# dcherednik/atracdenc

Hardware: AMD Instinct MI355X
Metric: ATRAC3 1024-sample stereo frames/sec (higher is better)
Workload: dtype f32; 1 GPU; ATRAC3 LP2 132 kbps stereo, 64 streams x 64 frames = 4096 frames per GPU per step (BASELINE configs[1]), 'noise' PCM resident in HBM, frames written to HBM (PCIe excluded); streams_per_gpu=64, frame_bytes=384, input=noise, tonal_components=True, parallelism=streams/1, launch=1 process x 1 GPU(s), one host thread and one at3hip context per device, collectives=none (no RCCL); start/stop barrier only

## Files before the change

atracdenc_amd/csrc/at3_k_gain.hpp:

```cpp
#pragma once
#include "at3_common.hpp"

namespace at3 {

struct GainParams {
    const float* sub;
    GainRec* rec;
    cpx* bins;
    BandState* state;
    Curve* curves;
    int n_blocks;
    int f0;
    int js;
    int n_streams;
    int literal;
};

constexpr int kLowCutBin = 38;

__device__ inline void median3_32(const float* in, float* out)
{
    for (int i = 0; i < 32; ++i) {
        const int lo = i > 0 ? i - 1 : 0;
        const int hi = i < 31 ? i + 1 : 31;
        if (hi - lo == 1) {
            out[i] = fmaxf(in[lo], in[hi]);
        } else {
            const float a = in[lo], b = in[lo + 1], c = in[hi];
            out[i] = fmaxf(fminf(a, b), fminf(fmaxf(a, b), c));
        }
    }
}

__device__ inline float curve_target(const float* in, const float* filtered)
{
    float maxRaw = 0.0f;
    for (int i = 0; i < 32; ++i) maxRaw = fmaxf(maxRaw, in[i]);
    float bestLevel = 0.0f;
    int bestEnd = -1;
    for (int j = 0; j + 3 <= 32; ++j) {
        const float minVal = fminf(fminf(filtered[j], filtered[j + 1]), filtered[j + 2]);
        if (minVal > bestLevel) {
            bestLevel = minVal;
            bestEnd = j + 2;
        }
    }
    float plateau = 0.0f;
    bool release = false;
    if (!(bestLevel < 1e-6f)) {
        plateau = bestLevel;
        while (bestEnd + 1 < 32 && filtered[bestEnd + 1] >= bestLevel) ++bestEnd;
        if (bestEnd < 31) {
            if (in[31] < bestLevel * 0.1f) {
                release = true;
            } else {
                bool anyHigh = false;
                for (int i = bestEnd + 1; i < 32; ++i)
                    if (in[i] >= bestLevel * 0.7f) {
                        anyHigh = true;
                        break;
                    }
                release = !anyHigh && (in[31] < bestLevel * 0.5f);
            }
        }
    }
    const bool usePlateau = plateau > 1e-6f && !release && plateau >= maxRaw * 0.4f;
    return usePlateau ? plateau : in[31];
}

__device__ __forceinline__ int irfft_pad(int i) { return i + (i >> 5); }

template <bool Z1>
__device__ __forceinline__ void bfly4_inv_sparse(f2& x0, f2& x1, f2& x2, f2& x3, f2 w1, f2 w3)
{
    const f2 s2 = pk_cmul(x3, w3);
    const f2 f0 = x0;
    if (Z1) {
        x2 = f0 - s2;
        x0 = f0 + s2;
        x1 = pk_sub_ib(f0, s2);
        x3 = pk_add_ib(f0, s2);
    } else {
        const f2 s0 = pk_cmul(x1, w1);
        const f2 s3 = s0 + s2, s4 = s0 - s2;
        x2 = f0 - s3;
        x0 = f0 + s3;
        x1 = pk_add_ib(f0, s4);
        x3 = pk_sub_ib(f0, s4);
    }
}

template <int KAPPA>
__device__ __forceinline__ void irfft_pass_2_8(cpx* F, const cpx* tw, int lane)
{
    cpx* B = F + 33 * lane + KAPPA;
    f2 x[16];
    const int r0 = (lane >> 4) + 4 * ((lane >> 2) & 3) + 16 * (lane & 3);
#pragma unroll
    for (int i = 0; i < 16; ++i) {
        const int r = r0 + 64 * (i >> 2);
        const bool nz = (i & 3) == 0 ? r >= 38 : (i & 3) == 1 ? r == 0 : (i & 3) == 3 ? r <= 218 : false;
        x[i] = f2{0.0f, 0.0f};
        if ((i & 3) != 2 && nz) x[i] = ld2(B + 2 * i);
    }
    const f2 a1 = ld2(tw + 256 * KAPPA), a3 = ld2(tw + 768 * KAPPA);
    bfly4_inv_sparse<false>(x[0], x[1], x[2], x[3], a1, a3);
#pragma unroll
    for (int g = 1; g < 4; ++g) bfly4_inv_sparse<true>(x[4 * g], x[4 * g + 1], x[4 * g + 2], x[4 * g + 3], a1, a3);
#pragma unroll
    for (int j = 0; j < 4; ++j) {
        const int k = KAPPA + 2 * j;
        bfly4<true>(x[j], x[j + 4], x[j + 8], x[j + 12], ld2(tw + 64 * k), ld2(tw + 128 * k), ld2(tw + 192 * k));
    }
#pragma unroll
    for (int i = 0; i < 16; ++i) st2(B + 2 * i, x[i]);
}

struct Tw32_128 {
    f2 a[3];
    f2 w[4][3];
};
__device__ __forceinline__ Tw32_128 irfft_tw_32_128(const cpx (*g)[128], int v)
{
    Tw32_128 t;
    t.a[0] = ld2(&g[0][v]);
    t.a[1] = ld2(&g[1][v]);
    t.a[2] = ld2(&g[2][v]);
#pragma unroll
    for (int j = 0; j < 4; ++j) {
        t.w[j][0] = ld2(&g[3 + 3 * j][v]);
        t.w[j][1] = ld2(&g[4 + 3 * j][v]);
        t.w[j][2] = ld2(&g[5 + 3 * j][v]);
    }
    return t;
}
__device__ __forceinline__ void irfft_pass_32_128(cpx* F, const Tw32_128& t, int v)
{
    const int k = v & 31, G2 = v >> 5;
    cpx* B = F + 528 * G2 + k;
    f2 x[16];
#pragma unroll
    for (int i = 0; i < 16; ++i) x[i] = ld2(B + 33 * i);
#pragma unroll
    for (int g = 0; g < 4; ++g) bfly4<true>(x[4 * g], x[4 * g + 1], x[4 * g + 2], x[4 * g + 3], t.a[0], t.a[1], t.a[2]);
#pragma unroll
    for (int j = 0; j < 4; ++j) bfly4<true>(x[j], x[j + 4], x[j + 8], x[j + 12], t.w[j][0], t.w[j][1], t.w[j][2]);
#pragma unroll
    for (int i = 0; i < 16; ++i) st2(B + 33 * i, x[i]);
}

template <int NT>
struct Tw512 {
    f2 w[512 / NT][3];
};
template <int NT>
__device__ __forceinline__ Tw512<NT> irfft_tw_512(const cpx (*g)[128], int tid)
{
    static_assert(NT == 128, "Tables::gain_tw is laid out for 128 work-items");
    Tw512<NT> t;
#pragma unroll
    for (int u = 0; u < 512 / NT; ++u) {
        t.w[u][0] = ld2(&g[15 + 3 * u][tid]);
        t.w[u][1] = ld2(&g[16 + 3 * u][tid]);
        t.w[u][2] = ld2(&g[17 + 3 * u][tid]);
    }
    return t;
}
template <int NT>
__device__ __forceinline__ void irfft_pass_512(cpx* F, const Tw512<NT>& t, int tid)
{
#pragma unroll
    for (int u0 = 0; u0 < 512 / NT; u0 += 4) {
        f2 x[4][4];
        cpx* B[4];
#pragma unroll
        for (int u = 0; u < 4; ++u) {
            B[u] = F + irfft_pad(tid + NT * (u0 + u));
#pragma unroll
            for (int q = 0; q < 4; ++q) x[u][q] = ld2(B[u] + 528 * q);
        }
#pragma unroll
        for (int u = 0; u < 4; ++u) bfly4<true>(x[u][0], x[u][1], x[u][2], x[u][3], t.w[u0 + u][0], t.w[u0 + u][1], t.w[u0 + u][2]);
#pragma unroll
        for (int u = 0; u < 4; ++u) {
            st2(B[u] + 528, x[u][1]);
            st2(B[u] + 1056, x[u][2]);
        }
    }
}

template <int CTRL>
__device__ __forceinline__ double dpp_f64_zero_fill(double v)
{
    const uint64_t b = (uint64_t)__double_as_longlong(v);
    const uint32_t lo = (uint32_t)AT3_DPP((uint32_t)b, CTRL, true), hi = (uint32_t)AT3_DPP((uint32_t)(b >> 32), CTRL, true);
    return __longlong_as_double((long long)(((uint64_t)hi << 32) | lo));
}
__device__ __forceinline__ double row_scan_add_f64(double v)
{
    v += dpp_f64_zero_fill<0x111>(v);
    v += dpp_f64_zero_fill<0x112>(v);
    v += dpp_f64_zero_fill<0x114>(v);
    v += dpp_f64_zero_fill<0x118>(v);
    return v;
}
constexpr int kGainBins = 220;

constexpr int kSpecRowStride = 18;
constexpr int kSpecItemBytes = 2432;
struct SpecItemLds {
    union {
        cpx x[16 * kSpecRowStride];
        double e[304];
    };
};
static_assert(sizeof(SpecItemLds) == kSpecItemBytes, "SpecItemLds layout");

__global__ __launch_bounds__(64) void k_gain_spec(GainParams p, const Tables* T, int n_items)
{
    __shared__ __attribute__((aligned(16))) SpecItemLds s_item[4];
    const int lane = threadIdx.x, row = lane >> 4, L = lane & 15;
    SpecItemLds& S = s_item[row];
    const int nfr = p.n_blocks - p.f0;
    const int quads = (nfr + 3) >> 2;
    int wg = blockIdx.x;
    const int band = wg % 3; wg /= 3;
    const int ch = wg % 2; wg /= 2;
    const int fr = 4 * (wg % quads) + row;
    const int s = wg / quads;
    const bool valid = fr < nfr;
    const int f = p.f0 + (valid ? fr : nfr - 1);
    const int item = (((s * nfr) + (f - p.f0)) * 2 + ch) * 3 + band;
    (void)n_items;
    const int cb = f - 1;
    const size_t sublen = (size_t)(p.n_blocks + 2) * 256;
    const float* sb0 = p.sub + ((size_t)s * 8 + 0 * 4 + band) * sublen + (size_t)(cb + 2) * 256 - 128;
    const float* sb1 = p.sub + ((size_t)s * 8 + 1 * 4 + band) * sublen + (size_t)(cb + 2) * 256 - 128;
    GainRec* rec = p.rec + (((size_t)s * p.n_blocks + f) * 2 + ch) * 3 + band;
    cpx* bins = p.bins + (size_t)item * kGainBins;

    f2 a[16];
    {
        f2 raw[16], rb[16], win[16];
#pragma unroll
        for (int t = 0; t < 16; ++t) {
            const int i = L + 16 * t;
            raw[t] = *reinterpret_cast<const f2*>((p.js || ch == 0 ? sb0 : sb1) + 2 * i);
            if (p.js) rb[t] = *reinterpret_cast<const f2*>(sb1 + 2 * i);
        }
#pragma unroll
        for (int t = 0; t < 16; ++t) win[t] = ld2(&T->spec16_win[t][L]);
        __builtin_amdgcn_sched_barrier(0);
#pragma unroll
        for (int t = 0; t < 16; ++t) {
            f2 v = raw[t];
            if (p.js) v = (ch == 0) ? (v + rb[t]) * mk2(0.5f, 0.5f) : (v - rb[t]) * mk2(0.5f, 0.5f);
            a[4 * (t & 3) + (t >> 2)] = v * win[t];
        }
    }
    f2 tw_l[15];
#pragma unroll
    for (int q = 0; q < 15; ++q) tw_l[q] = ld2(&T->spec16_tw[q][L]);
    __builtin_amdgcn_sched_barrier(0);
    {
        const f2 w0 = ld2(&T->tw256[0]);
#pragma unroll
        for (int q3 = 0; q3 < 4; ++q3) bfly4<false>(a[4 * q3], a[4 * q3 + 1], a[4 * q3 + 2], a[4 * q3 + 3], w0, w0, w0);
#pragma unroll
        for (int k = 0; k < 4; ++k)
            bfly4<false>(a[k], a[k + 4], a[k + 8], a[k + 12], ld2(&T->tw256[16 * k]), ld2(&T->tw256[32 * k]), ld2(&T->tw256[48 * k]));
    }
    f2 b[16];
    {
#pragma unroll
        for (int r = 0; r < 16; ++r) st2(&S.x[r * kSpecRowStride + L], a[r]);
        wave_sync();
        const float4* src = reinterpret_cast<const float4*>(&S.x[L * kSpecRowStride]);
#pragma unroll
        for (int m = 0; m < 8; ++m) {
            const float4 v = src[m];
            b[2 * m] = mk2(v.x, v.y);
            b[2 * m + 1] = mk2(v.z, v.w);
        }
        wave_sync();
    }
    {
        const f2 u1 = tw_l[0], u2 = tw_l[1], u3 = tw_l[2];
#pragma unroll
        for (int q1 = 0; q1 < 4; ++q1) bfly4<false>(b[q1], b[q1 + 4], b[q1 + 8], b[q1 + 12], u1, u2, u3);
#pragma unroll
        for (int j = 0; j < 4; ++j) bfly4<false>(b[4 * j], b[4 * j + 1], b[4 * j + 2], b[4 * j + 3], tw_l[3 + 3 * j], tw_l[4 + 3 * j], tw_l[5 + 3 * j]);
    }
    f2 fa[8], fb[8];
    f2 f128 = mk2(0.0f, 0.0f);
    {
        const int partner = 4 * ((lane & 48) | ((16 - L) & 15));
#pragma unroll
        for (int jj = 0; jj < 8; ++jj) {
            const int je = 15 - jj;
            const f2 pe = b[(je >> 2) + 4 * (je & 3)];
            f2 other;
            other.x = __uint_as_float((uint32_t)__builtin_amdgcn_ds_bpermute(partner, (int)__float_as_uint(pe.x)));
            other.y = __uint_as_float((uint32_t)__builtin_amdgcn_ds_bpermute(partner, (int)__float_as_uint(pe.y)));
            if (jj > 0) {
                const int j0 = 16 - jj;
                const f2 own = b[(j0 >> 2) + 4 * (j0 & 3)];
                if (L == 0) other = own;
            }
            const f2 fpk = b[(jj >> 2) + 4 * (jj & 3)];
            const cpx stw = T->spec16_stw[jj][L];
            const float fnr = other.x, fni = -other.y;
            const float f1r = fpk.x + fnr, f1i = fpk.y + fni;
            const float f2r = fpk.x - fnr, f2i = fpk.y - fni;
            const float twr = f2r * stw.r - f2i * stw.i, twi = f2r * stw.i + f2i * stw.r;
            fa[jj] = mk2((f1r + twr) * 0.5f, (f1i + twi) * 0.5f);
            fb[jj] = mk2((f1r - twr) * 0.5f, (twi - f1i) * 0.5f);
        }
        if (L == 0) {
            const f2 f0 = b[0];
            fa[0] = mk2(f0.x + f0.y, 0.0f);
            fb[0] = mk2(f0.x - f0.y, 0.0f);
        }
        {
            const f2 fpk = b[2];
            const cpx stw = T->spec16_stw[8][L];
            const float fnr = fpk.x, fni = -fpk.y;
            const float f1r = fpk.x + fnr, f1i = fpk.y + fni;
            const float f2r = fpk.x - fnr, f2i = fpk.y - fni;
            const float twr = f2r * stw.r - f2i * stw.i, twi = f2r * stw.i + f2i * stw.r;
            f128 = mk2((f1r - twr) * 0.5f, (twi - f1i) * 0.5f);
        }
    }
    if (valid) {
#pragma unroll
        for (int jj = 0; jj < 8; ++jj) {
            const int k = L + 16 * jj;
            if (k >= kLowCutBin) st2(&bins[k - kLowCutBin], fa[jj]);
            st2(&bins[256 - k - kLowCutBin], fb[jj]);
        }
        if (L == 0) st2(&bins[128 - kLowCutBin], f128);
    }
    bool fast_done = false;
    {
        const double h1 = (double)T->hpf_w[1], h2 = (double)T->hpf_w[2];
        double et = 0.0, ef = 0.0;
#pragma unroll
        for (int jj = 0; jj < 8; ++jj) {
            const int k = L + 16 * jj;
            const double ea = (double)fa[jj].x * fa[jj].x + (double)fa[jj].y * fa[jj].y;
            const double eb = (double)fb[jj].x * fb[jj].x + (double)fb[jj].y * fb[jj].y;
            et += ea;
            et += eb;
            const double wa = (k < kLowCutBin) ? 0.0 : (k == kLowCutBin) ? ea * h1 * h1 : (k == kLowCutBin + 1) ? ea * h2 * h2 : ea;
            ef += wa;
            ef += eb;
        }
        if (L == 0) {
            const double e128 = (double)f128.x * f128.x + (double)f128.y * f128.y;
            et += e128;
            ef += e128;
        }
        et = row_scan_add_f64(et);
        ef = row_scan_add_f64(ef);
        bool need = false;
        float hfr = 0.0f;
        if (L == 15) {
            if (et > 0.0 && ef > 0.0) {
                const double r = ef / et;
                hfr = (float)r;
                if (!(hfr >= 1e-30f)) {
                    need = true;
                } else {
                    const uint32_t hb = __float_as_uint(hfr);
                    const double below = ((double)__uint_as_float(hb - 1u) + (double)hfr) * 0.5, above = ((double)hfr + (double)__uint_as_float(hb + 1u)) * 0.5;
                    const double margin = r * 4e-13;
                    need = !(r - below > margin && above - r > margin);
                }
            }
        }
        if (p.literal || __ballot(need && valid) != 0ull) {
            fast_done = false;
        } else {
            if (valid && L == 15) rec->hfr = hfr;
            fast_done = true;
        }
    }
    if (fast_done) return;
    {
#pragma unroll
        for (int jj = 0; jj < 8; ++jj) {
            const int k = L + 16 * jj;
            S.e[k] = (double)fa[jj].x * fa[jj].x + (double)fa[jj].y * fa[jj].y;
            S.e[256 - k] = (double)fb[jj].x * fb[jj].x + (double)fb[jj].y * fb[jj].y;
        }
        if (L == 0) S.e[128] = (double)f128.x * f128.x + (double)f128.y * f128.y;
        for (int k = 257 + L; k < 304; k += 16) S.e[k] = 0.0;
    }
    wave_sync();
    double acc = 0.0;
    if (lane < 8) {
        const int it = lane >> 1, kind = lane & 1;
        const double* E = s_item[it].e;
        const double h1 = (double)T->hpf_w[1], h2 = (double)T->hpf_w[2];
        if (kind == 1) {
            acc += E[kLowCutBin] * h1 * h1;
            acc += E[kLowCutBin + 1] * h2 * h2;
        }
        const double* src = E + (kind ? kLowCutBin + 2 : 0);
        for (int k0 = 0; k0 < 256; k0 += 16) {
            double v[16];
#pragma unroll
            for (int i = 0; i < 16; ++i) v[i] = src[k0 + i];
#pragma unroll
            for (int i = 0; i < 16; ++i) acc += v[i];
        }
        acc += src[256];
    }
    const uint64_t ab = (uint64_t)__double_as_longlong(acc);
    const int alo = (int)(uint32_t)ab, ahi = (int)(uint32_t)(ab >> 32);
    const uint64_t fb64 = (uint64_t)(uint32_t)__builtin_amdgcn_ds_bpermute(4 * (2 * row + 1), alo) |
                          ((uint64_t)(uint32_t)__builtin_amdgcn_ds_bpermute(4 * (2 * row + 1), ahi) << 32);
    const uint64_t tb64 = (uint64_t)(uint32_t)__builtin_amdgcn_ds_bpermute(4 * (2 * row), alo) |
                          ((uint64_t)(uint32_t)__builtin_amdgcn_ds_bpermute(4 * (2 * row), ahi) << 32);
    if (valid && L == 0) {
        const double totalE = __longlong_as_double((long long)tb64), filtE = __longlong_as_double((long long)fb64);
        rec->hfr = (totalE > 0.0) ? (float)(filtE / totalE) : 0.0f;
    }
}

struct GainLds {
    cpx f[2048 + 64];
};

__global__ __launch_bounds__(128) void k_gain_analysis(GainParams p, const Tables* __restrict__ T)
{
    __shared__ __attribute__((aligned(16))) GainLds s_item[1];
    const int tid = threadIdx.x, wave = __builtin_amdgcn_readfirstlane((int)(threadIdx.x >> 6)), lane = threadIdx.x & 63;
    GainLds& L = s_item[0];
    const int nfr = p.n_blocks - p.f0;
    const bool valid = true;
    int wg = blockIdx.x;
    const size_t item = blockIdx.x;
    const int band = wg % 3; wg /= 3;
    const int ch = wg % 2; wg /= 2;
    const int f = p.f0 + wg % nfr;
    const int s = wg / nfr;
    GainRec* rec = p.rec + (((size_t)s * p.n_blocks + f) * 2 + ch) * 3 + band;
    const float hfr = rec->hfr;
    const cpx* bins = p.bins + item * kGainBins;
    const int k0 = kLowCutBin + tid, k1 = kLowCutBin + 128 + tid;
    const cpx bin0 = bins[tid];
    const cpx bin1 = bins[k1 <= 256 ? 128 + tid : tid];
    const cpx stw_in0 = T->stw2048[k0 - 1];
    const cpx stw_in1 = T->stw2048[k1 - 1 < 1024 ? k1 - 1 : 1023];
    const float hpf1 = T->hpf_w[1], hpf2 = T->hpf_w[2];
    __builtin_amdgcn_sched_barrier(0);
    if (hfr < 0.05f) return;
    __builtin_amdgcn_sched_barrier(0);
    const Tw32_128 tw_b = irfft_tw_32_128(T->gain_tw, tid);
    const Tw512<128> tw_c = irfft_tw_512<128>(T->gain_tw, tid);
    __builtin_amdgcn_sched_barrier(0);
#pragma unroll
    for (int q = 0; q < 2; ++q) {
        const int k = q ? k1 : k0;
        const cpx fr = q ? bin1 : bin0;
        cpx fk;
        const float scale = 8.0f;
        if (k == 256) {
            fk.r = fr.r * scale * 0.5f;
            fk.i = 0.0f;
        } else if (k >= kLowCutBin + 2) {
            fk.r = fr.r * scale;
            fk.i = fr.i * scale;
        } else {
            const float w = (k == kLowCutBin) ? hpf1 : hpf2;
            fk.r = fr.r * scale * w;
            fk.i = fr.i * scale * w;
        }
        const cpx fok = cmul(fk, q ? stw_in1 : stw_in0);
        cpx a, b, nb;
        a.r = fk.r + fok.r; a.i = fk.i + fok.i;
        b.r = fk.r - fok.r; b.i = -(fk.i - fok.i);
        nb.r = 0.0f - b.r; nb.i = 0.0f - b.i;
        if (k <= 256) {
            const int pa = fft_leaf_pos<2048>(k);
            L.f[irfft_pad(pa)] = a;
            L.f[irfft_pad(pa) + 1] = a;
            const int pb = fft_leaf_pos<2048>(2048 - k);
            L.f[irfft_pad(pb) - 1] = b;
            L.f[irfft_pad(pb)] = nb;
        }
    }
    __syncthreads();

    if (wave == 0) irfft_pass_2_8<0>(L.f, T->tw2048, lane);
    else irfft_pass_2_8<1>(L.f, T->tw2048, lane);
    __syncthreads();

    irfft_pass_32_128(L.f, tw_b, tid);
    __syncthreads();

    irfft_pass_512<128>(L.f, tw_c, tid);
    __syncthreads();


    const float norm = 1.0f / 4096.0f;
    float* s_micro = reinterpret_cast<float*>(L.f);
#pragma unroll
    for (int q = 0; q < 2; ++q) {
        const int n = tid + 128 * q;
        const int c = (n & 3) | ((n & 0xc) << 1) | ((n & 0x10) >> 2) | (n & 0xe0);
        cpx* src = L.f + 528 + 4 * c + (c >> 3);
        float acc = 0.0f;
#pragma unroll
        for (int i = 0; i < 4; ++i) {
            const f2 v = ld2(src + i) * norm;
            const f2 sq = v * v;
            st2(src + i, sq);
            acc += sq.x;
            acc += sq.y;
        }
        acc /= 8;
        s_micro[c] = sqrtf(acc);
    }
    __syncthreads();
    if (tid < 32) {
        const cpx* src = L.f + 528 + 33 * lane;
        f2 x[32];
#pragma unroll
        for (int i = 0; i < 32; ++i) x[i] = ld2(src + i);
        float acc = 0.0f;
#pragma unroll
        for (int i = 0; i < 32; ++i) {
            acc += x[i].x;
            acc += x[i].y;
        }
        acc /= 64;
        rec->gain[lane] = sqrtf(acc);
    } else if (wave == 1 && lane < 32) {
        const float4 ma = *reinterpret_cast<const float4*>(s_micro + 8 * lane), mb = *reinterpret_cast<const float4*>(s_micro + 8 * lane + 4);
        float m[8] = {ma.x, ma.y, ma.z, ma.w, mb.x, mb.y, mb.z, mb.w};
#pragma unroll
        for (int i = 1; i < 8; ++i) {
#pragma unroll
            for (int k = i; k > 0; --k) {
                const float lo = fminf(m[k - 1], m[k]), hi = fmaxf(m[k - 1], m[k]);
                m[k - 1] = lo;
                m[k] = hi;
            }
        }
        rec->lo[lane] = m[2];
        rec->hi[lane] = m[6];
    }
}

constexpr int kGa1RowStride = 18;
constexpr int kGa1RowSlots = 16 * kGa1RowStride + 16;
constexpr int kGa1SubStride = 33;
struct Gain1Lds {
    union {
        cpx x[4 * kGa1RowSlots];
        struct {
            cpx out[32 * kGa1SubStride];
            float micro[256];
        };
    };
};
static_assert(sizeof(Gain1Lds) <= 10240, "sixteen items per CU");

struct PermPair {
    int a, b;
};
__device__ __forceinline__ PermPair perm32_swap(int a, int b)
{
    const auto r = __builtin_amdgcn_permlane32_swap(a, b, false, false);
    return PermPair{(int)r[0], (int)r[1]};
}
__device__ __forceinline__ PermPair perm16_swap(int a, int b)
{
    const auto r = __builtin_amdgcn_permlane16_swap(a, b, false, false);
    return PermPair{(int)r[0], (int)r[1]};
}
template <bool WIDE>
__device__ __forceinline__ void swap_f2(f2& a, f2& b)
{
    const PermPair x = WIDE ? perm32_swap((int)__float_as_uint(a.x), (int)__float_as_uint(b.x)) : perm16_swap((int)__float_as_uint(a.x), (int)__float_as_uint(b.x));
    const PermPair y = WIDE ? perm32_swap((int)__float_as_uint(a.y), (int)__float_as_uint(b.y)) : perm16_swap((int)__float_as_uint(a.y), (int)__float_as_uint(b.y));
    a = mk2(__uint_as_float((uint32_t)x.a), __uint_as_float((uint32_t)y.a));
    b = mk2(__uint_as_float((uint32_t)x.b), __uint_as_float((uint32_t)y.b));
}

__global__ __launch_bounds__(64) AT3_WAVES_PER_EU(4) void k_gain_analysis1(GainParams p, const Tables* T)
{
    __shared__ __attribute__((aligned(16))) Gain1Lds L;
    const int lane = threadIdx.x, R = lane >> 4, j = lane & 15;
    const int nfr = p.n_blocks - p.f0;
    int wg = blockIdx.x;
    const size_t item = blockIdx.x;
    const int band = wg % 3; wg /= 3;
    const int ch = wg % 2; wg /= 2;
    const int f = p.f0 + wg % nfr;
    const int s = wg / nfr;
    GainRec* rec = p.rec + (((size_t)s * p.n_blocks + f) * 2 + ch) * 3 + band;
    const float hfr = rec->hfr;
    if (hfr < 0.05f) return;
    const cpx* bins = p.bins + item * kGainBins;
    const cpx* tw = T->tw2048;

#define AT3_STAGE() __builtin_amdgcn_sched_barrier(0)
    const int r0 = (lane >> 4) + 4 * ((lane >> 2) & 3) + 16 * (lane & 3);
    cpx ba[4], bb[4], sa[4], sb[4], b256 = {0.0f, 0.0f}, s256 = {0.0f, 0.0f};
#pragma unroll
    for (int q = 0; q < 4; ++q) {
        const int ka = r0 + 64 * q, kb = 256 - r0 - 64 * q;
        const int kac = ka >= kLowCutBin ? ka : kLowCutBin, kbc = kb >= kLowCutBin ? kb : kLowCutBin;
        ba[q] = bins[kac - kLowCutBin];
        sa[q] = T->stw2048[kac - 1];
        bb[q] = bins[kbc - kLowCutBin];
        sb[q] = T->stw2048[kbc - 1];
    }
    if (lane == 0) {
        b256 = bins[256 - kLowCutBin];
        s256 = T->stw2048[255];
    }
    const float hpf1 = T->hpf_w[1], hpf2 = T->hpf_w[2];
    f2 a1[2], a3[2], w8[2][4][3];
#pragma unroll
    for (int kappa = 0; kappa < 2; ++kappa) {
        a1[kappa] = ld2(tw + 256 * kappa);
        a3[kappa] = ld2(tw + 768 * kappa);
#pragma unroll
        for (int jj = 0; jj < 4; ++jj) {
            const int k = kappa + 2 * jj;
            w8[kappa][jj][0] = ld2(tw + 64 * k);
            w8[kappa][jj][1] = ld2(tw + 128 * k);
            w8[kappa][jj][2] = ld2(tw + 192 * k);
        }
    }
    f2 twb[15];
#pragma unroll
    for (int sl = 0; sl < 15; ++sl) twb[sl] = ld2(&T->ga1_twb[0][sl][j]);
    AT3_STAGE();
    f2 la[4], lb[4], la256 = mk2(0.0f, 0.0f);
    {
        auto leaf = [&](cpx fr, cpx stw, int k, bool want_b) -> f2 {
            cpx fk;
            const float scale = 8.0f;
            if (k == 256) {
                fk.r = fr.r * scale * 0.5f;
                fk.i = 0.0f;
            } else if (k >= kLowCutBin + 2) {
                fk.r = fr.r * scale;
                fk.i = fr.i * scale;
            } else {
                const float w = (k == kLowCutBin) ? hpf1 : hpf2;
                fk.r = fr.r * scale * w;
                fk.i = fr.i * scale * w;
            }
            const cpx fok = cmul(fk, stw);
            return want_b ? mk2(fk.r - fok.r, -(fk.i - fok.i)) : mk2(fk.r + fok.r, fk.i + fok.i);
        };
#pragma unroll
        for (int q = 0; q < 4; ++q) {
            const int ka = r0 + 64 * q, kb = 256 - r0 - 64 * q;
            la[q] = (ka >= kLowCutBin) ? leaf(ba[q], sa[q], ka, false) : mk2(0.0f, 0.0f);
            lb[q] = (kb >= kLowCutBin) ? leaf(bb[q], sb[q], kb, true) : mk2(0.0f, 0.0f);
        }
        if (lane == 0) la256 = leaf(b256, s256, 256, false);
    }
    f2 y[2][16];
    f2 twc[2][4][3];
#pragma unroll
    for (int kappa = 0; kappa < 2; ++kappa) {
        f2 x[16];
#pragma unroll
        for (int i = 0; i < 16; ++i) x[i] = mk2(0.0f, 0.0f);
#pragma unroll
        for (int q = 0; q < 4; ++q) {
            x[4 * q] = la[q];
            x[4 * q + 3] = kappa ? mk2(0.0f - lb[q].x, 0.0f - lb[q].y) : lb[q];
        }
        x[1] = la256;
        bfly4_inv_sparse<false>(x[0], x[1], x[2], x[3], a1[kappa], a3[kappa]);
#pragma unroll
        for (int g = 1; g < 4; ++g) bfly4_inv_sparse<true>(x[4 * g], x[4 * g + 1], x[4 * g + 2], x[4 * g + 3], a1[kappa], a3[kappa]);
#pragma unroll
        for (int jj = 0; jj < 4; ++jj) bfly4<true>(x[jj], x[jj + 4], x[jj + 8], x[jj + 12], w8[kappa][jj][0], w8[kappa][jj][1], w8[kappa][jj][2]);
        cpx* row = L.x + R * kGa1RowSlots;
#pragma unroll
        for (int i = 0; i < 16; ++i) st2(row + i * kGa1RowStride + j, x[i]);
        wave_sync();
        f2 b[16];
        {
            const float4* src = reinterpret_cast<const float4*>(row + j * kGa1RowStride);
#pragma unroll
            for (int m = 0; m < 8; ++m) {
                const float4 v = src[m];
                b[2 * m] = mk2(v.x, v.y);
                b[2 * m + 1] = mk2(v.z, v.w);
            }
        }
        wave_sync();
#pragma unroll
        for (int g = 0; g < 4; ++g) bfly4<true>(b[4 * g], b[4 * g + 1], b[4 * g + 2], b[4 * g + 3], twb[0], twb[1], twb[2]);
#pragma unroll
        for (int jj = 0; jj < 4; ++jj) bfly4<true>(b[jj], b[jj + 4], b[jj + 8], b[jj + 12], twb[3 + 3 * jj], twb[4 + 3 * jj], twb[5 + 3 * jj]);
#pragma unroll
        for (int i = 0; i < 16; ++i) y[kappa][i] = b[i];
        AT3_STAGE();
        if (kappa == 0) {
#pragma unroll
            for (int sl = 0; sl < 15; ++sl) twb[sl] = ld2(&T->ga1_twb[1][sl][j]);
        } else {
#pragma unroll
            for (int u = 0; u < 2; ++u)
#pragma unroll
                for (int t = 0; t < 4; ++t)
#pragma unroll
                    for (int q = 0; q < 3; ++q) twc[u][t][q] = ld2(&T->ga1_twc[4 * u + t][q][lane]);
        }
        AT3_STAGE();
    }
#pragma unroll
    for (int u = 0; u < 2; ++u)
#pragma unroll
        for (int t = 0; t < 8; ++t) swap_f2<true>(y[u][t], y[u][8 + t]);
#pragma unroll
    for (int u = 0; u < 2; ++u)
#pragma unroll
        for (int t = 0; t < 4; ++t) {
            swap_f2<false>(y[u][t], y[u][4 + t]);
            swap_f2<false>(y[u][8 + t], y[u][12 + t]);
        }
#pragma unroll
    for (int u = 0; u < 2; ++u)
#pragma unroll
        for (int t = 0; t < 4; ++t) {
            const int i = 4 * R + t;
            bfly4<true>(y[u][t], y[u][4 + t], y[u][8 + t], y[u][12 + t], twc[u][t][0], twc[u][t][1], twc[u][t][2]);
            st2(L.out + kGa1SubStride * i + 2 * j + u, y[u][4 + t]);
            st2(L.out + kGa1SubStride * (16 + i) + 2 * j + u, y[u][8 + t]);
        }
    wave_sync();
    const float norm = 1.0f / 4096.0f;
#pragma unroll
    for (int q = 0; q < 4; ++q) {
        const int n = lane + 64 * q;
        const int c = (n & 3) | ((n & 0xc) << 1) | ((n & 0x10) >> 2) | (n & 0xe0);
        const cpx* src = L.out + 4 * c + (c >> 3);
        float acc = 0.0f;
#pragma unroll
        for (int i = 0; i < 4; ++i) {
            const f2 v = ld2(src + i) * norm;
            const f2 sq = v * v;
            acc += sq.x;
            acc += sq.y;
        }
        acc /= 8;
        L.micro[c] = sqrtf(acc);
    }
    wave_sync();
    if (lane < 32) {
        const cpx* src = L.out + kGa1SubStride * lane;
        f2 x[32];
#pragma unroll
        for (int i = 0; i < 32; ++i) x[i] = ld2(src + i);
        float acc = 0.0f;
#pragma unroll
        for (int i = 0; i < 32; ++i) {
            const f2 v = x[i] * norm;
            const f2 sq = v * v;
            acc += sq.x;
            acc += sq.y;
        }
        acc /= 64;
        rec->gain[lane] = sqrtf(acc);
    } else {
        const int sf = lane - 32;
        const float4 ma = *reinterpret_cast<const float4*>(L.micro + 8 * sf), mb = *reinterpret_cast<const float4*>(L.micro + 8 * sf + 4);
        float m[8] = {ma.x, ma.y, ma.z, ma.w, mb.x, mb.y, mb.z, mb.w};
#pragma unroll
        for (int i = 1; i < 8; ++i) {
#pragma unroll
            for (int k = i; k > 0; --k) {
                const float lo = fminf(m[k - 1], m[k]), hi = fmaxf(m[k - 1], m[k]);
                m[k - 1] = lo;
                m[k] = hi;
            }
        }
        rec->lo[sf] = m[2];
        rec->hi[sf] = m[6];
    }
}

__global__ __launch_bounds__(256) void k_gain_tail(GainParams p, int n_items)
{
    __shared__ float s_g[8][32], s_f[8][32], s_m[8][32];
    const int tid = threadIdx.x, grp = tid >> 5, j = tid & 31, half = grp & 1;
    const int nfr = p.n_blocks - p.f0;
    int item = blockIdx.x * 8 + grp;
    const bool valid = item < n_items;
    if (!valid) item = n_items - 1;
    int wg = item;
    const int band = wg % 3; wg /= 3;
    const int ch = wg % 2; wg /= 2;
    const int f = p.f0 + wg % nfr;
    const int s = wg / nfr;
    GainRec* rec = p.rec + (((size_t)s * p.n_blocks + f) * 2 + ch) * 3 + band;
    const float hfr = rec->hfr;
    const float g_j = rec->gain[j];
    asm volatile("" ::"v"(g_j));
    const bool active = valid && !(hfr < 0.05f);
    if (__ballot(active) == 0ull) return;
    float* s_gain = s_g[grp];
    float* s_filt = s_f[grp];
    float* s_minv = s_m[grp];
    const float in_j = active ? g_j : 0.0f;
    s_gain[j] = in_j;
    wave_sync();
    float filt_j;
    {
        const float a = s_gain[j > 0 ? j - 1 : 0], c = s_gain[j < 31 ? j + 1 : 31];
        if (j == 0) filt_j = fmaxf(in_j, c);
        else if (j == 31) filt_j = fmaxf(a, in_j);
        else filt_j = fmaxf(fminf(a, in_j), fminf(fmaxf(a, in_j), c));
    }
    s_filt[j] = filt_j;
    wave_sync();
    s_minv[j] = (j <= 29) ? fminf(fminf(filt_j, s_filt[j < 30 ? j + 1 : 31]), s_filt[j < 30 ? j + 2 : 31]) : -1.0f;
    wave_sync();
    float maxRaw = 0.0f, sum = 0.0f, bestLevel = 0.0f;
    int bestEnd = -1;
    for (int k = 0; k < 32; ++k) {
        const float g = s_gain[k];
        maxRaw = fmaxf(maxRaw, g);
        sum += g;
        const float mv = s_minv[k];
        if (k <= 29 && mv > bestLevel) {
            bestLevel = mv;
            bestEnd = k + 2;
        }
    }
    const uint32_t ge = (uint32_t)(__ballot(filt_j >= bestLevel) >> (32 * half));
    const uint32_t high = (uint32_t)(__ballot(in_j >= bestLevel * 0.7f) >> (32 * half));
// ... 505 lines not shown
```

atracdenc_amd/csrc/at3_tables.cpp:

```cpp
#include "at3_tables.hpp"
#include "at1_tables.hpp"
#include "at3p_tables.hpp"

#include <cmath>
#include <cstring>

#define AT3_RUNTIME_LIBM __attribute__((optnone, noinline))

namespace at3 {

extern const float kTapHalf[24];
const float kTapHalf[24] = {
    -0.00001461907,  -0.00009205479, -0.000056157569, 0.00030117269, 0.0002422519,  -0.00085293897,
    -0.0005205574,   0.0020340169,   0.00078333891,   -0.0042153862, -0.00075614988, 0.0078402944,
    -0.000061169922, -0.01344162,    0.0024626821,    0.021736089,   -0.007801671,   -0.034090221,
    0.01880949,      0.054326009,    -0.043596379,    -0.099384367,  0.13207909,     0.46424159};

namespace {

#include "at3_libm64.inc"

const short kAthMilliBel[] = {
    9669, 9669, 9626, 9512, 9353, 9113, 8882, 8676, 8469, 8243, 7997, 7748, 7492, 7239, 7000, 6762, 6529, 6302, 6084, 5900,
    5717, 5534, 5351, 5167, 5004, 4812, 4638, 4466, 4310, 4173, 4050, 3922, 3723, 3577, 3451, 3281, 3132, 3036, 2902, 2760,
    2658, 2591, 2441, 2301, 2212, 2125, 2018, 1900, 1770, 1682, 1594, 1512, 1430, 1341, 1260, 1198, 1136, 1057, 998,  943,
    887,  846,  744,  712,  693,  668,  637,  606,  580,  555,  529,  502,  475,  448,  422,  398,  375,  351,  327,  322,
    312,  301,  291,  268,  246,  215,  182,  146,  107,  61,   13,   -35,  -96,  -156, -179, -235, -295, -350, -401, -421,
    -446, -499, -532, -535, -513, -476, -431, -313, -179, 8,    203,  403,  580,  736,  881,  1022, 1154, 1251, 1348, 1421,
    1479, 1399, 1285, 1193, 1287, 1519, 1914, 2369, 3352, 4352, 5352, 6352, 7352, 8352, 9352, 9999, 9999, 9999, 9999, 9999};

const uint16_t kBfuStart[33] = {0,   8,   16,  24,  32,  40,  48,  56,  64,  80,  96,  112, 128, 144, 160, 176, 192,
                                224, 256, 288, 320, 352, 384, 416, 448, 480, 512, 576, 640, 704, 768, 896, 1024};

}

AT3_RUNTIME_LIBM float ath_db(float freq)
{
    if (freq < 10.) freq = 10.;
    if (freq > 29853.) freq = 29853.;
    const double fl = 40. * log10(0.1 * freq);
    const unsigned idx = (unsigned)fl;
    return 0.01 * (kAthMilliBel[idx] * (1 + idx - fl) + kAthMilliBel[idx + 1] * (fl - idx));
}

AT3_RUNTIME_LIBM void fill_twiddles(cpx* tw, int n, bool inverse)
{
    const double pi = 3.141592653589793238462643383279502884197169399375105820974944;
    for (int i = 0; i < n; ++i) {
        double phase = -2 * pi * i / n;
        if (inverse) phase *= -1;
        tw[i].r = (float)cos(phase);
        tw[i].i = (float)sin(phase);
    }
}

AT3_RUNTIME_LIBM void mdct_sincos(float* dst, size_t n, float scale)
{
    const float alpha = 2.0 * M_PI / (8.0 * n);
    const float omiga = 2.0 * M_PI / n;
    scale = sqrtf(scale / n);
    for (size_t i = 0; i < (n >> 2); ++i) {
        dst[2 * i + 0] = scale * cosf(omiga * i + alpha);
        dst[2 * i + 1] = scale * sinf(omiga * i + alpha);
    }
}

namespace {

AT3_RUNTIME_LIBM void fill_super_twiddles(cpx* tw, int ncfft, bool inverse)
{
    for (int i = 0; i < ncfft / 2; ++i) {
        double phase = -3.14159265358979323846264338327 * ((double)(i + 1) / ncfft + .5);
        if (inverse) phase *= -1;
        tw[i].r = (float)cos(phase);
        tw[i].i = (float)sin(phase);
    }
}

}

AT3_RUNTIME_LIBM void build_tables(Tables* t)
{
    memset(t, 0, sizeof(*t));
    for (int i = 0; i < 24; ++i) t->qmf_win[i] = t->qmf_win[47 - i] = kTapHalf[i] * 2.0;
    for (uint32_t i = 0; i < 64; ++i) t->scale[i] = pow(2.0, (double)(i / 3.0 - 21.0));
    for (int i = 0; i < 256; ++i) t->enc_win[i] = (sin(((i + 0.5) / 256.0 - 0.5) * M_PI) + 1.0);
    for (int i = 0; i < 16; ++i) t->gain_level[i] = pow(2.0, 4 - i);
    for (int i = 0; i < 31; ++i) t->gain_interp[i] = pow(2.0, -1.0 / 8 * (i - 15));

    mdct_sincos(t->mdct_sincos, 512, 1.0f);
    fill_twiddles(t->tw128, 128, false);
    fill_twiddles(t->tw256, 256, false);
    fill_twiddles(t->tw2048, 2048, true);
    fill_super_twiddles(t->stw256, 256, false);
    fill_super_twiddles(t->stw2048, 2048, true);
    for (int L = 0; L < 16; ++L) {
        for (int q = 1; q <= 3; ++q) t->spec16_tw[q - 1][L] = t->tw256[4 * q * L];
        for (int j = 0; j < 4; ++j)
            for (int q = 1; q <= 3; ++q) t->spec16_tw[3 + 3 * j + q - 1][L] = t->tw256[q * (L + 16 * j)];
        for (int jj = 0; jj < 9; ++jj) {
            const int k = L + 16 * jj;
            cpx z = {0.0f, 0.0f};
            if (k >= 1 && k <= 128 && (jj < 8 || L == 0)) z = t->stw256[k - 1];
            t->spec16_stw[jj][L] = z;
        }
    }
    for (int tid = 0; tid < 128; ++tid) {
        const int k = tid & 31;
        for (int q = 0; q < 3; ++q) t->gain_tw[q][tid] = t->tw2048[16 * (q + 1) * k];
        for (int j = 0; j < 4; ++j)
            for (int q = 0; q < 3; ++q) t->gain_tw[3 + 3 * j + q][tid] = t->tw2048[4 * (q + 1) * (k + 32 * j)];
        for (int u = 0; u < 4; ++u)
            for (int q = 0; q < 3; ++q) t->gain_tw[15 + 3 * u + q][tid] = t->tw2048[(q + 1) * (tid + 128 * u)];
    }

    for (int u = 0; u < 2; ++u)
        for (int j = 0; j < 16; ++j) {
            const int k = 2 * j + u;
            for (int q = 0; q < 3; ++q) t->ga1_twb[u][q][j] = t->tw2048[16 * (q + 1) * k];
            for (int jj = 0; jj < 4; ++jj)
                for (int q = 0; q < 3; ++q) t->ga1_twb[u][3 + 3 * jj + q][j] = t->tw2048[4 * (q + 1) * (k + 32 * jj)];
        }
    for (int lane = 0; lane < 64; ++lane)
        for (int u = 0; u < 2; ++u)
            for (int tt = 0; tt < 4; ++tt) {
                const int kk = 2 * (lane & 15) + u + 32 * (4 * (lane >> 4) + tt);
                for (int q = 0; q < 3; ++q) t->ga1_twc[4 * u + tt][q][lane] = t->tw2048[(q + 1) * kk];
            }

    for (int en = 0; en < 18; ++en)
        for (int L = 0; L < 16; ++L) {
            const int q1 = L >> 2, q2 = L & 3, b = q1 + 4 * q2;
            float* v = t->mdct_tab[en][L];
            if (en < 4) {
                const int e = 2 * b + 32 * en;
                v[0] = t->enc_win[e]; v[1] = t->enc_win[128 + e]; v[2] = t->enc_win[127 - e]; v[3] = t->enc_win[255 - e];
            } else if (en < 8) {
                const int n = 2 * (b + 16 * (en - 4));
                v[0] = t->mdct_sincos[n]; v[1] = t->mdct_sincos[n + 1]; v[2] = t->mdct_sincos[n + 128]; v[3] = t->mdct_sincos[n + 129];
            } else if (en < 12) {
                const int n = 2 * (8 * q1 + 2 * q2 + 32 * (en - 8));
                v[0] = t->mdct_sincos[n]; v[1] = t->mdct_sincos[n + 1]; v[2] = t->mdct_sincos[n + 2]; v[3] = t->mdct_sincos[n + 3];
            } else if (en < 15) {
                const int j = en - 11, k = 2 * q2;
                v[0] = t->tw128[4 * j * k].r; v[1] = t->tw128[4 * j * k].i; v[2] = t->tw128[4 * j * (k + 1)].r; v[3] = t->tw128[4 * j * (k + 1)].i;
            } else {
                const int j = en - 14, k = 8 * q1 + 2 * q2;
                v[0] = t->tw128[j * k].r; v[1] = t->tw128[j * k].i; v[2] = t->tw128[j * (k + 1)].r; v[3] = t->tw128[j * (k + 1)].i;
            }
        }

    {
        const float eN = 0.15f * 512.0f;
        const float fN = 512.0f;
        for (int n = 0; n < 512; ++n) {
            const float fn = (float)n;
            if (n == 0) {
                t->planck[n] = 0.0f;
            } else if (fn < eN) {
                const float z = eN * (1.0f / fn + 1.0f / (fn - eN));
                t->planck[n] = 1.0f / (1.0f + expf(z));
            } else if (fn <= fN - eN) {
                t->planck[n] = 1.0f;
            } else {
                const float m = fN - fn;
                const float z = eN * (1.0f / m + 1.0f / (m - eN));
                t->planck[n] = 1.0f / (1.0f + expf(z));
            }
        }
        for (int i = 0; i < 3; ++i) t->hpf_w[i] = 0.5f * (1.0f - cosf((float)M_PI * i / 2.0f));
    }
    for (int L = 0; L < 16; ++L)
        for (int tt = 0; tt < 16; ++tt) {
            const int i = L + 16 * tt;
            t->spec16_win[tt][L].r = t->planck[2 * i];
            t->spec16_win[tt][L].i = t->planck[2 * i + 1];
        }

    for (size_t i = 0; i < 1024; ++i) {
        float f = (float)(i + 3) * 0.5 * 44100 / (float)1024;
        float v = log10f(f) - 3.5;
        v = -10 * v * v + 3 - f / 3000;
        v = pow(10, (0.1 * v));
        t->loud_curve[i] = v;
    }
    {
        float ath_line[1024];
        const float mf = (float)44100 / 2000.0;
        for (size_t i = 0; i < 1024; ++i) {
            const float f = (float)(i + 1) * mf / 1024;
            float trh = ath_db(1.e3 * f) - 100;
            trh -= f * f * 0.015;
            ath_line[i] = trh;
        }
        for (int b = 0; b < 32; ++b) {
            float x = 999;
            for (int line = kBfuStart[b]; line < kBfuStart[b + 1]; ++line) x = fminf(x, ath_line[line]);
            x = pow(10, 0.1f * x);
            t->ath_bfu[b] = x;
        }
    }
    static const double tab[16][2] = {
        {0x1.661ec79f8f3bep+0, -0x1.efec65b963019p-2}, {0x1.571ed4aaf883dp+0, -0x1.b0b6832d4fca4p-2},
        {0x1.49539f0f010b0p+0, -0x1.7418b0a1fb77bp-2}, {0x1.3c995b0b80385p+0, -0x1.39de91a6dcf7bp-2},
        {0x1.30d190c8864a5p+0, -0x1.01d9bf3f2b631p-2}, {0x1.25e227b0b8ea0p+0, -0x1.97c1d1b3b7af0p-3},
        {0x1.1bb4a4a1a343fp+0, -0x1.2f9e393af3c9fp-3}, {0x1.12358f08ae5bap+0, -0x1.960cbbf788d5cp-4},
        {0x1.0953f419900a7p+0, -0x1.a6f9db6475fcep-5}, {0x1.0000000000000p+0, 0x0.0p+0},
        {0x1.e608cfd9a47acp-1, 0x1.338ca9f24f53dp-4},  {0x1.ca4b31f026aa0p-1, 0x1.476a9543891bap-3},
        {0x1.b2036576afce6p-1, 0x1.e840b4ac4e4d2p-3},  {0x1.9c2d163a1aa2dp-1, 0x1.40645f0c6651cp-2},
        {0x1.886e6037841edp-1, 0x1.88e9c2c1b9ff8p-2},  {0x1.767dcf5534862p-1, 0x1.ce0a44eb17bccp-2}};
    static const double poly[4] = {-0x1.712b6f70a7e4dp-2, 0x1.ecabf496832e0p-2, -0x1.715479ffae3dep-1,
                                   0x1.715475f35c8b8p+0};
    memcpy(t->log2f_tab, tab, sizeof(tab));
    memcpy(t->log2f_poly, poly, sizeof(poly));
    memcpy(t->libm.log_c, kLogData, sizeof(t->libm.log_c));
    memcpy(t->libm.log_tab, kLogData + 18, sizeof(t->libm.log_tab));
    memcpy(t->libm.exp_c, kExpData, sizeof(t->libm.exp_c));
    memcpy(t->libm.exp_tab, kExpTab, sizeof(t->libm.exp_tab));
}

}

namespace at1 {

namespace {

const uint16_t kSpecsStartLong[kMaxBfus] = {0,   8,   16,  24,  32,  36,  40,  44,  48,  56,  64,  72,  80,  86,  92,  98,  104, 110,
                                            116, 122, 128, 134, 140, 146, 152, 159, 166, 173, 180, 189, 198, 207, 216, 226, 236, 246,
                                            256, 268, 280, 292, 304, 316, 328, 340, 352, 372, 392, 412, 432, 452, 472, 492};
const uint8_t kSpecsPerBlock[kMaxBfus] = {8,  8,  8,  8,  4,  4,  4,  4,  8,  8,  8,  8,  6,  6,  6,  6,  6,  6,
                                          6,  6,  6,  6,  6,  6,  7,  7,  7,  7,  9,  9,  9,  9,  10, 10, 10, 10,
                                          12, 12, 12, 12, 12, 12, 12, 12, 20, 20, 20, 20, 20, 20, 20, 20};

}

AT3_RUNTIME_LIBM void build_tables(Tables* t)
{
    memset(t, 0, sizeof(*t));
    for (int i = 0; i < 24; ++i) t->qmf_win[i] = t->qmf_win[47 - i] = at3::kTapHalf[i] * 2.0;
    for (uint32_t i = 0; i < 64; ++i) t->scale[i] = pow(2.0, (double)(i / 3.0 - 21.0));
    for (uint32_t i = 0; i < 32; ++i) t->sine[i] = sin((i + 0.5) * (M_PI / (2.0 * 32.0)));
    at3::mdct_sincos(t->sc512, 512, 1.0f);
    at3::mdct_sincos(t->sc256, 256, 0.5f);
    at3::mdct_sincos(t->sc64, 64, 0.5f);
    at3::fill_twiddles(t->tw128, 128, false);
    at3::fill_twiddles(t->tw64, 64, false);
    at3::fill_twiddles(t->tw16, 16, false);
    for (size_t i = 0; i < 512; ++i) {
        float f = (float)(i + 3) * 0.5 * 44100 / (float)512;
        float v = log10f(f) - 3.5;
        v = -10 * v * v + 3 - f / 3000;
        v = pow(10, (0.1 * v));
        t->loud[i] = v;
    }
    {
        float ath_line[512];
        const float mf = (float)44100 / 2000.0;
        for (size_t i = 0; i < 512; ++i) {
            const float f = (float)(i + 1) * mf / 512;
            float trh = at3::ath_db(1.e3 * f) - 100;
            trh -= f * f * 0.015;
            ath_line[i] = trh;
        }
        for (int b = 0; b < kMaxBfus; ++b) {
            float x = 999;
            for (int line = kSpecsStartLong[b]; line < kSpecsStartLong[b] + kSpecsPerBlock[b]; ++line) x = fmin(x, ath_line[line]);
            x = pow(10, 0.1 * x);
            t->ath_bfu[b] = x;
        }
    }
    static const float fir[10] = {-8.65163e-18 * 2.0, -0.00851586 * 2.0, -6.74764e-18 * 2.0, 0.0209036 * 2.0, -3.36639e-17 * 2.0,
                                  -0.0438162 * 2.0,   -1.54175e-17 * 2.0, 0.0931738 * 2.0,   -5.52212e-17 * 2.0, -0.313819 * 2.0};
    memcpy(t->fir, fir, sizeof(fir));
    static const float fix_long[kMaxBfus] = {7, 7, 7, 6, 6, 6, 6, 6, 6, 6, 6, 6, 6, 6, 6, 6, 6, 6, 6, 6, 6, 6, 5, 5, 5, 5,
                                             5, 5, 5, 5, 5, 5, 5, 5, 5, 4, 4, 4, 3, 3, 3, 3, 3, 3, 2, 1, 1, 1, 1, 0, 0, 0};
    static const float fix_short[kMaxBfus] = {6, 6, 6, 6, 6, 6, 6, 6, 6, 6, 6, 6, 6, 6, 6, 6, 6, 6, 6, 6, 6, 6, 6, 6, 5, 5,
                                              5, 5, 5, 5, 5, 5, 5, 5, 5, 5, 4, 4, 4, 4, 4, 4, 4, 4, 0, 0, 0, 0, 0, 0, 0, 0};
    memcpy(t->fix_long, fix_long, sizeof(fix_long));
    memcpy(t->fix_short, fix_short, sizeof(fix_short));
    static const double tab[16][2] = {
        {0x1.661ec79f8f3bep+0, -0x1.57bf7808caadep-2}, {0x1.571ed4aaf883dp+0, -0x1.2bef0a7c06ddbp-2},
        {0x1.49539f0f010b0p+0, -0x1.01eae7f513a67p-2}, {0x1.3c995b0b80385p+0, -0x1.b31d8a68224e9p-3},
        {0x1.30d190c8864a5p+0, -0x1.6574f0ac07758p-3}, {0x1.25e227b0b8ea0p+0, -0x1.1aa2bc79c8100p-3},
        {0x1.1bb4a4a1a343fp+0, -0x1.a4e76ce8c0e5ep-4}, {0x1.12358f08ae5bap+0, -0x1.1973c5a611cccp-4},
        {0x1.0953f419900a7p+0, -0x1.252f438e10c1ep-5}, {0x1.0000000000000p+0, 0x0.0p+0},
        {0x1.e608cfd9a47acp-1, 0x1.aa5aa5df25984p-5},  {0x1.ca4b31f026aa0p-1, 0x1.c5e53aa362eb4p-4},
        {0x1.b2036576afce6p-1, 0x1.526e57720db08p-3},  {0x1.9c2d163a1aa2dp-1, 0x1.bc2860d224770p-3},
        {0x1.886e6037841edp-1, 0x1.1058bc8a07ee1p-2},  {0x1.767dcf5534862p-1, 0x1.4043057b6ee09p-2}};
    memcpy(t->logf_tab, tab, sizeof(tab));
    t->logf_ln2 = 0x1.62e42fefa39efp-1;
    t->logf_poly[0] = -0x1.00ea348b88334p-2;
    t->logf_poly[1] = 0x1.5575b0be00b6ap-2;
    t->logf_poly[2] = -0x1.ffffef20a4123p-2;
}

}

namespace at3p {

namespace {

const float kFir[384] = {
#include "at3p_fir.inc"
};

}

AT3_RUNTIME_LIBM void build_tables(Tables* t)
{
    memset(t, 0, sizeof(*t));
    memcpy(t->fir, kFir, sizeof(kFir));
    const float dct_scale = 32.0 * (float)(128 * 512.0);
    at3::mdct_sincos(t->sc32, 32, dct_scale / 2);
    at3::mdct_sincos(t->sc256, 256, 1.0f);
    at3::fill_twiddles(t->tw8, 8, false);
    at3::fill_twiddles(t->tw64, 64, false);
    for (size_t i = 0; i < 128; i++) t->sine128[i] = 2.0 * sinf((i + 0.5) * (M_PI / (2.0 * 128)));
    for (size_t i = 0; i < 64; i++) t->sine64[i] = 2.0 * sinf((i + 0.5) * (M_PI / (2.0 * 64)));
}

}
```

Measured before the change: 15.99 million frames/s.

## Fuse final radix-4 IFFT pass with power/micro-RMS computation in gain kernel

Remaps the last radix-4 inverse-FFT pass so each work-item owns the four contiguous outputs of one micro chunk. It then squares, normalises and reduces them to the micro RMS in registers, instead of storing the pass results and reloading them after a barrier. This drops one __syncthreads and a round of LDS reads. The twiddle table is permuted on the host to match, and micro values go to a scattered LDS location, so the median reader now uses eight scalar loads in place of two float4 loads.

```diff
diff --git a/atracdenc_amd/csrc/at3_k_gain.hpp b/atracdenc_amd/csrc/at3_k_gain.hpp
--- a/atracdenc_amd/csrc/at3_k_gain.hpp
+++ b/atracdenc_amd/csrc/at3_k_gain.hpp
@@ -149,43 +149,52 @@
     for (int i = 0; i < 16; ++i) st2(B + 33 * i, x[i]);
 }
 
-template <int NT>
+__device__ __forceinline__ int gain_chunk_of(int n) { return (n & 3) | ((n & 0xc) << 1) | ((n & 0x10) >> 2) | (n & 0xe0); }
+
 struct Tw512 {
-    f2 w[512 / NT][3];
+    f2 w[4][3];
 };
-template <int NT>
-__device__ __forceinline__ Tw512<NT> irfft_tw_512(const cpx (*g)[128], int tid)
-{
-    static_assert(NT == 128, "Tables::gain_tw is laid out for 128 work-items");
-    Tw512<NT> t;
-#pragma unroll
-    for (int u = 0; u < 512 / NT; ++u) {
+__device__ __forceinline__ Tw512 irfft_tw_512(const cpx (*g)[128], int tid)
+{
+    Tw512 t;
+#pragma unroll
+    for (int u = 0; u < 4; ++u) {
         t.w[u][0] = ld2(&g[15 + 3 * u][tid]);
         t.w[u][1] = ld2(&g[16 + 3 * u][tid]);
         t.w[u][2] = ld2(&g[17 + 3 * u][tid]);
     }
     return t;
 }
-template <int NT>
-__device__ __forceinline__ void irfft_pass_512(cpx* F, const Tw512<NT>& t, int tid)
-{
-#pragma unroll
-    for (int u0 = 0; u0 < 512 / NT; u0 += 4) {
-        f2 x[4][4];
-        cpx* B[4];
+__device__ __forceinline__ int gain_micro_at(int c)
+{
+    const int cc = c & 127, hi = c >> 7;
+    return 2 * (1584 * hi + 4 * cc + (cc >> 3)) + (((cc >> 2) & 1) ^ hi);
+}
+__device__ __forceinline__ void irfft_pass_512_squares(cpx* F, const Tw512& t, int c)
+{
+    cpx* B = F + 4 * c + (c >> 3);
+    f2 x[4][4];
+#pragma unroll
+    for (int u = 0; u < 4; ++u)
+#pragma unroll
+        for (int q = 0; q < 4; ++q) x[u][q] = ld2(B + u + 528 * q);
+#pragma unroll
+    for (int u = 0; u < 4; ++u) bfly4<true>(x[u][0], x[u][1], x[u][2], x[u][3], t.w[u][0], t.w[u][1], t.w[u][2]);
+    const float norm = 1.0f / 4096.0f;
+    float* micro = reinterpret_cast<float*>(F);
+#pragma unroll
+    for (int h = 0; h < 2; ++h) {
+        float acc = 0.0f;
 #pragma unroll
         for (int u = 0; u < 4; ++u) {
-            B[u] = F + irfft_pad(tid + NT * (u0 + u));
-#pragma unroll
-            for (int q = 0; q < 4; ++q) x[u][q] = ld2(B[u] + 528 * q);
-        }
-#pragma unroll
-        for (int u = 0; u < 4; ++u) bfly4<true>(x[u][0], x[u][1], x[u][2], x[u][3], t.w[u0 + u][0], t.w[u0 + u][1], t.w[u0 + u][2]);
-#pragma unroll
-        for (int u = 0; u < 4; ++u) {
-            st2(B[u] + 528, x[u][1]);
-            st2(B[u] + 1056, x[u][2]);
-        }
+            const f2 v = x[u][1 + h] * norm;
+            const f2 sq = v * v;
+            st2(B + u + 528 * (1 + h), sq);
+            acc += sq.x;
+            acc += sq.y;
+        }
+        acc /= 8;
+        micro[gain_micro_at(c + 128 * h)] = sqrtf(acc);
     }
 }
 
@@ -458,7 +467,7 @@
     if (hfr < 0.05f) return;
     __builtin_amdgcn_sched_barrier(0);
     const Tw32_128 tw_b = irfft_tw_32_128(T->gain_tw, tid);
-    const Tw512<128> tw_c = irfft_tw_512<128>(T->gain_tw, tid);
+    const Tw512 tw_c = irfft_tw_512(T->gain_tw, tid);
     __builtin_amdgcn_sched_barrier(0);
 #pragma unroll
     for (int q = 0; q < 2; ++q) {
@@ -500,29 +509,7 @@
     irfft_pass_32_128(L.f, tw_b, tid);
     __syncthreads();
 
-    irfft_pass_512<128>(L.f, tw_c, tid);
-    __syncthreads();
-
-
-    const float norm = 1.0f / 4096.0f;
-    float* s_micro = reinterpret_cast<float*>(L.f);
-#pragma unroll
-    for (int q = 0; q < 2; ++q) {
-        const int n = tid + 128 * q;
-        const int c = (n & 3) | ((n & 0xc) << 1) | ((n & 0x10) >> 2) | (n & 0xe0);
-        cpx* src = L.f + 528 + 4 * c + (c >> 3);
-        float acc = 0.0f;
-#pragma unroll
-        for (int i = 0; i < 4; ++i) {
-            const f2 v = ld2(src + i) * norm;
-            const f2 sq = v * v;
-            st2(src + i, sq);
-            acc += sq.x;
-            acc += sq.y;
-        }
-        acc /= 8;
-        s_micro[c] = sqrtf(acc);
-    }
+    irfft_pass_512_squares(L.f, tw_c, gain_chunk_of(tid));
     __syncthreads();
     if (tid < 32) {
         const cpx* src = L.f + 528 + 33 * lane;
@@ -538,8 +525,10 @@
         acc /= 64;
         rec->gain[lane] = sqrtf(acc);
     } else if (wave == 1 && lane < 32) {
-        const float4 ma = *reinterpret_cast<const float4*>(s_micro + 8 * lane), mb = *reinterpret_cast<const float4*>(s_micro + 8 * lane + 4);
-        float m[8] = {ma.x, ma.y, ma.z, ma.w, mb.x, mb.y, mb.z, mb.w};
+        const float* s_micro = reinterpret_cast<const float*>(L.f);
+        float m[8];
+#pragma unroll
+        for (int i = 0; i < 8; ++i) m[i] = s_micro[gain_micro_at(8 * lane + i)];
 #pragma unroll
         for (int i = 1; i < 8; ++i) {
 #pragma unroll
diff --git a/atracdenc_amd/csrc/at3_tables.cpp b/atracdenc_amd/csrc/at3_tables.cpp
--- a/atracdenc_amd/csrc/at3_tables.cpp
+++ b/atracdenc_amd/csrc/at3_tables.cpp
@@ -110,8 +110,9 @@
         for (int q = 0; q < 3; ++q) t->gain_tw[q][tid] = t->tw2048[16 * (q + 1) * k];
         for (int j = 0; j < 4; ++j)
             for (int q = 0; q < 3; ++q) t->gain_tw[3 + 3 * j + q][tid] = t->tw2048[4 * (q + 1) * (k + 32 * j)];
+        const int c = (tid & 3) | ((tid & 0xc) << 1) | ((tid & 0x10) >> 2) | (tid & 0xe0);
         for (int u = 0; u < 4; ++u)
-            for (int q = 0; q < 3; ++q) t->gain_tw[15 + 3 * u + q][tid] = t->tw2048[(q + 1) * (tid + 128 * u)];
+            for (int q = 0; q < 3; ++q) t->gain_tw[15 + 3 * u + q][tid] = t->tw2048[(q + 1) * (4 * c + u)];
     }
 
     for (int u = 0; u < 2; ++u)
```

Result: slower. 15.80 million frames/s (-1.2%).
